# Deci-AI/super-gradients

Measured on NVIDIA H100. Metric: images/sec YOLO-NAS-S 640 bf16 train, higher is better.
Workload: dtype bf16

## Files before the change

### super_gradients_b200/csrc/conv_sm100.cu

```cuda
#include <cuda.h>

#include <cstdlib>
#include <cstring>

#include "common.cuh"
#include "conv_sm100.h"
#include "sm100_host.h"
#include "sm100_ptx.cuh"

namespace sm100 {

constexpr int BLOCK_M = 128;
constexpr int NUM_THREADS = 384;
constexpr int CONSUMER_THREADS = 256;
constexpr int MAX_STAGES = 8;

struct Params {
  int M;
  int N;
  int C;
  int KC;
  int n_tiles;
  int stages;
  int P, Q;
  int stride, pad;
  int b_cols_per_tap;
  int ntaps;
  signed char tap_dh[9], tap_dw[9], tap_b[9];
  int out_mode, o_mul, oh_add, ow_add, outH, outW;
  long long y_pitch;
  int y_off;
  bf16* y;
  const float* scale;
  const float* shift;
  const bf16* residual;
  double* stats;
  int stats_repl;
  int act;
};

__device__ __forceinline__ long long out_row(const Params& p, long long m) {
  if (p.out_mode == 0) return m;
  const int pq = p.P * p.Q;
  const int n = (int)(m / pq);
  const int rem = (int)(m - (long long)n * pq);
  const int j = rem / p.Q, i = rem - j * p.Q;
  return ((long long)n * p.outH + j * p.o_mul + p.oh_add) * p.outW + i * p.o_mul + p.ow_add;
}

__device__ __forceinline__ void consumer_sync() { asm volatile("bar.sync 1, %0;" ::"n"(CONSUMER_THREADS) : "memory"); }

constexpr uint32_t CTRL_BAR_BYTES = 16u * MAX_STAGES;

template <int BN>
__global__ void __launch_bounds__(NUM_THREADS, 1)
conv_wgmma_kernel(const __grid_constant__ CUtensorMap map_a, const __grid_constant__ CUtensorMap map_b, const Params p) {
  SGB_GRID_DEP_LAUNCH();
  extern __shared__ __align__(1024) unsigned char smem_raw[];
  const uint32_t smem_base = (smem_u32(smem_raw) + 1023u) & ~1023u;
  const uint32_t a_bytes = BLOCK_M * p.KC * 2, b_bytes = BN * p.KC * 2;
  const uint32_t stage_bytes = a_bytes + ((b_bytes + 1023u) & ~1023u);
  const uint32_t ctrl = smem_base + p.stages * stage_bytes;
  auto full_bar = [&](int s) { return ctrl + 8u * s; };
  auto empty_bar = [&](int s) { return ctrl + 8u * (MAX_STAGES + s); };
  float* s_part = reinterpret_cast<float*>(smem_raw + (ctrl + CTRL_BAR_BYTES - smem_u32(smem_raw)));
  float* s_stats = s_part + 8 * 2 * BN;

  const int warp = threadIdx.x >> 5, lane = threadIdx.x & 31;
  const int m_tiles = (p.M + BLOCK_M - 1) / BLOCK_M;
  const int total_tiles = m_tiles * p.n_tiles;
  const int chunks = (p.C + p.KC - 1) / p.KC;
  const int k_iters = p.ntaps * chunks;

  if (threadIdx.x == 0) {
    for (int s = 0; s < p.stages; ++s) {
      mbar_init(full_bar(s), 1);
      mbar_init(empty_bar(s), 8);
    }
    asm volatile("fence.mbarrier_init.release.cluster;" ::: "memory");
    asm volatile("fence.proxy.async.shared::cta;" ::: "memory");
  }
  if (p.stats)
    for (int i = threadIdx.x; i < 2 * p.N; i += NUM_THREADS) s_stats[i] = 0.f;
  __syncthreads();
  SGB_GRID_DEP_WAIT();

  if (warp == 0) {
    if (elect_one()) {
      int stg = 0;
      uint32_t par = 1;
      const int pq = p.P * p.Q;
// ... 75 lines not shown
        rrow[h] = p.residual ? p.residual + orow * p.y_pitch + p.y_off + n0 : nullptr;
      }
#pragma unroll
      for (int j = 0; j < BN / 8; ++j) {
        const int col = 8 * j + 2 * (lane & 3);
        const bool col_ok = col < ncols;
        float sum0 = 0.f, sum1 = 0.f, sq0 = 0.f, sq1 = 0.f;
#pragma unroll
        for (int h = 0; h < 2; ++h) {
          float v0 = acc[4 * j + 2 * h], v1 = acc[4 * j + 2 * h + 1];
          const bool ok = row_ok[h] && col_ok;
          if (p.scale && col_ok) {
            v0 *= p.scale[n0 + col];
            v1 *= p.scale[n0 + col + 1];
          }
          if (p.shift && col_ok) {
            v0 += p.shift[n0 + col];
            v1 += p.shift[n0 + col + 1];
          }
          if (rrow[h] && ok) {
            const uint32_t rr = *reinterpret_cast<const uint32_t*>(rrow[h] + col);
            v0 += __uint_as_float(rr << 16);
            v1 += __uint_as_float(rr & 0xffff0000u);
          }
          if (p.act != SGB_ACT_NONE) {
            v0 = apply_act(v0, p.act);
            v1 = apply_act(v1, p.act);
          }
          __nv_bfloat162 hh = __floats2bfloat162_rn(v0, v1);
          const uint32_t pk = *reinterpret_cast<uint32_t*>(&hh);
          if (ok) {
            *reinterpret_cast<uint32_t*>(yrow[h] + col) = pk;
            const float lo = __uint_as_float(pk << 16), hi = __uint_as_float(pk & 0xffff0000u);
            sum0 += lo;
            sum1 += hi;
            sq0 = fmaf(lo, lo, sq0);
            sq1 = fmaf(hi, hi, sq1);
          }
        }
        if (p.stats) {
#pragma unroll
          for (int o = 4; o < 32; o <<= 1) {
            sum0 += __shfl_xor_sync(0xffffffffu, sum0, o);
            sum1 += __shfl_xor_sync(0xffffffffu, sum1, o);
            sq0 += __shfl_xor_sync(0xffffffffu, sq0, o);
            sq1 += __shfl_xor_sync(0xffffffffu, sq1, o);
          }
          if (lane < 4) {
            float* part = s_part + (wg * 4 + wq) * 2 * BN;
            part[col] = sum0;
            part[col + 1] = sum1;
            part[BN + col] = sq0;
            part[BN + col + 1] = sq1;
          }
        }
      }
      if (p.stats) {
        consumer_sync();
        for (int i = threadIdx.x - 128; i < 2 * BN; i += CONSUMER_THREADS) {
          const int which = i / BN, c = i - which * BN;
          if (c < ncols) {
            float v = 0.f;
#pragma unroll
            for (int w = 0; w < 8; ++w) v += s_part[w * 2 * BN + i];
            s_stats[which * p.N + n0 + c] += v;
          }
        }
        consumer_sync();
      }
    }
  }
  __syncthreads();
  if (p.stats) {
    double* st = p.stats + (long long)(blockIdx.x & (p.stats_repl - 1)) * 2 * p.N;
    for (int i = threadIdx.x; i < 2 * p.N; i += NUM_THREADS) {
      const float v = s_stats[i];
      if (v != 0.f) atomicAdd(&st[i], (double)v);
    }
  }
}

struct WParams {
  int K, C;
  int R, S, stride, pad, P, Q;
  int npix;
  int CB;
  int n_ctiles, n_ktiles;
  int pix_per_cta;
  int stages;
  int cpad;
  float* dw;
};
constexpr int WPIX = 64;

template <int NB>
__global__ void __launch_bounds__(NUM_THREADS, 1)
wgrad_wgmma_kernel(const __grid_constant__ CUtensorMap map_dy, const __grid_constant__ CUtensorMap map_x, const WParams p) {
  SGB_GRID_DEP_LAUNCH();
  extern __shared__ __align__(1024) unsigned char smem_raw[];
  const uint32_t smem_base = (smem_u32(smem_raw) + 1023u) & ~1023u;
  const uint32_t a_bytes = 2 * WPIX * 128;
  const uint32_t b_box = WPIX * p.CB * 2;
  const int boxes = NB / p.CB;
  const uint32_t stage_bytes = a_bytes + (uint32_t)boxes * b_box;
  const uint32_t ctrl = smem_base + p.stages * stage_bytes;
  auto full_bar = [&](int s) { return ctrl + 8u * s; };
  auto empty_bar = [&](int s) { return ctrl + 8u * (MAX_STAGES + s); };

  const int warp = threadIdx.x >> 5, lane = threadIdx.x & 31;
  int w = blockIdx.x;
  const int ktile = w % p.n_ktiles; w /= p.n_ktiles;
  const int ctile = w % p.n_ctiles; w /= p.n_ctiles;
  const int tap = w % (p.R * p.S); w /= p.R * p.S;
  const int split = w;
  const int pix0 = split * p.pix_per_cta;
  const int pix1 = min(pix0 + p.pix_per_cta, p.npix);
  const int n_iters = (pix1 - pix0 + WPIX - 1) / WPIX;

  if (threadIdx.x == 0) {
    for (int s = 0; s < p.stages; ++s) {
      mbar_init(full_bar(s), 1);
      mbar_init(empty_bar(s), 8);
    }
    asm volatile("fence.mbarrier_init.release.cluster;" ::: "memory");
    asm volatile("fence.proxy.async.shared::cta;" ::: "memory");
  }
  __syncthreads();
  SGB_GRID_DEP_WAIT();

  if (n_iters > 0) {
    if (warp == 0) {
      if (elect_one()) {
        const int pq = p.P * p.Q;
        const int r = tap / p.S, s = tap - r * p.S;
        int stg = 0;
        uint32_t par = 1;
        for (int it = 0; it < n_iters; ++it) {
          mbar_wait(empty_bar(stg), par);
          const uint32_t sa = smem_base + stg * stage_bytes, sb = sa + a_bytes;
          mbar_expect_tx(full_bar(stg), a_bytes + (uint32_t)boxes * b_box);
          const int pix = pix0 + it * WPIX;
          tma_load_2d(sa, &map_dy, full_bar(stg), ktile * 128, pix);
          tma_load_2d(sa + WPIX * 128, &map_dy, full_bar(stg), ktile * 128 + 64, pix);
          const int n_img = pix / pq;
          const int rem = pix - n_img * pq;
          const int p0 = rem / p.Q, q0 = rem - p0 * p.Q;
          const int w0 = q0 * p.stride - p.pad, h0 = p0 * p.stride - p.pad;
          for (int bx = 0; bx < boxes; ++bx)
            tma_load_im2col_4d(sb + (uint32_t)bx * b_box, &map_x, full_bar(stg), ctile * NB + bx * p.CB, w0, h0, n_img, (uint16_t)s,
                               (uint16_t)r);
          if (++stg == p.stages) {
            stg = 0;
            par ^= 1;
          }
        }
      }
    } else if (warp >= 4) {
      const int wg = (warp >> 2) - 1, wq = warp & 3;
      const int b_row_bytes = p.CB * 2;
      float acc[NB / 2];
      int stg = 0, prev = -1;
      uint32_t par = 0;
      for (int it = 0; it < n_iters; ++it) {
        mbar_wait(full_bar(stg), par);
        const uint32_t sa = smem_base + stg * stage_bytes + (uint32_t)wg * (WPIX * 128), sb = smem_base + stg * stage_bytes + a_bytes;
        wgmma_fence();
#pragma unroll
        for (int j = 0; j < WPIX / 16; ++j) {
          const uint64_t da = smem_desc(sa + (uint32_t)j * 16u * 128u, 128, WPIX * 128, 8 * 128);
          const uint64_t db = smem_desc(sb + (uint32_t)j * 16u * (uint32_t)b_row_bytes, b_row_bytes, b_box, 8u * (uint32_t)b_row_bytes);
          mma_mn<NB>(acc, da, db, (it | j) != 0);
        }
        wgmma_commit();
        if (prev >= 0) {
          wgmma_wait<1>();
          __syncwarp();
          if (lane == 0) mbar_arrive(empty_bar(prev));
        }
        prev = stg;
        if (++stg == p.stages) {
          stg = 0;
          par ^= 1;
        }
      }
      wgmma_wait<0>();
      fence_regs(acc);
      const int row_len = p.R * p.S * p.cpad;
#pragma unroll
      for (int h = 0; h < 2; ++h) {
        const int ko = ktile * 128 + wg * 64 + wq * 16 + (lane >> 2) + 8 * h;
        if (ko < p.K) {
          float* drow = p.dw + (long long)ko * row_len + tap * p.cpad + ctile * NB + 2 * (lane & 3);
#pragma unroll
          for (int j = 0; j < NB / 8; ++j)
            asm volatile("red.global.add.v2.f32 [%0], {%1, %2};" ::"l"(drow + 8 * j), "f"(acc[4 * j + 2 * h]), "f"(acc[4 * j + 2 * h + 1])
                         : "memory");
        }
      }
    }
  }
}

EncodeTiledFn g_tiled = nullptr;
EncodeIm2colFn g_im2col = nullptr;
int g_num_sms = 0;
long long g_launches = 0;
long long launch_count() { return g_launches; }

int init_driver() {
  if (g_tiled && g_im2col) return SGB_OK;
  cudaDriverEntryPointQueryResult qres;
  void* fn = nullptr;
  if (cudaGetDriverEntryPoint("cuTensorMapEncodeTiled", &fn, cudaEnableDefault, &qres) != cudaSuccess || !fn) {
    sgb_set_error("cuTensorMapEncodeTiled entry point not found");
    return SGB_E_CUDA;
  }
  g_tiled = (EncodeTiledFn)fn;
  fn = nullptr;
  if (cudaGetDriverEntryPoint("cuTensorMapEncodeIm2col", &fn, cudaEnableDefault, &qres) != cudaSuccess || !fn) {
    sgb_set_error("cuTensorMapEncodeIm2col entry point not found");
    return SGB_E_CUDA;
  }
  g_im2col = (EncodeIm2colFn)fn;
  int dev = 0;
  cudaGetDevice(&dev);
  cudaDeviceGetAttribute(&g_num_sms, cudaDevAttrMultiProcessorCount, dev);
  return SGB_OK;
}

CUtensorMapSwizzle swizzle_for(int kc) {
  return kc == 64 ? CU_TENSOR_MAP_SWIZZLE_128B : (kc == 32 ? CU_TENSOR_MAP_SWIZZLE_64B : CU_TENSOR_MAP_SWIZZLE_32B);
}

bool enabled() {
  static int v = -1;
  if (v < 0) {
    const char* e = getenv("SGB_DISABLE_SM100");
    v = (e && e[0] == '1') ? 0 : 1;
  }
  return v == 1;
}

bool supported(const Problem& q) {
  if (!enabled()) return false;
  if (q.C % 16 != 0 || q.b_rows % 8 != 0) return false;
  if (!((q.R == 1 && q.S == 1) || (q.R == 3 && q.S == 3))) return false;
  if (q.stride != 1 && q.stride != 2) return false;
  if (q.a_pitch % 8 != 0 || q.y_pitch % 8 != 0 || q.y_off % 8 != 0) return false;
  if (((uintptr_t)q.a & 15) || ((uintptr_t)q.b & 15) || ((uintptr_t)q.y & 15)) return false;
  if ((long long)q.N * q.P * q.Q >= (1ll << 31)) return false;
  if (q.b_rows > 4096) return false;
  return true;
}

namespace {

template <class Fn>
struct Variant {
  int bn;
  Fn fn;
  int regs;
  bool ready;
};
typedef void (*ConvFn)(const CUtensorMap, const CUtensorMap, const Params);
typedef void (*WgradFn)(const CUtensorMap, const CUtensorMap, const WParams);
Variant<ConvFn> g_conv[] = {{16, conv_wgmma_kernel<16>, 0, false},   {32, conv_wgmma_kernel<32>, 0, false},
                            {48, conv_wgmma_kernel<48>, 0, false},   {64, conv_wgmma_kernel<64>, 0, false},
                            {96, conv_wgmma_kernel<96>, 0, false},   {128, conv_wgmma_kernel<128>, 0, false}};
Variant<WgradFn> g_wgrad[] = {{16, wgrad_wgmma_kernel<16>, 0, false}, {32, wgrad_wgmma_kernel<32>, 0, false},
                              {48, wgrad_wgmma_kernel<48>, 0, false}, {64, wgrad_wgmma_kernel<64>, 0, false},
                              {96, wgrad_wgmma_kernel<96>, 0, false}, {128, wgrad_wgmma_kernel<128>, 0, false}};

template <class Fn>
int prepare(Variant<Fn>& v, const char* what) {
  if (v.ready) return SGB_OK;
  if (int rc = sgb_cuda_check(cudaFuncSetAttribute(v.fn, cudaFuncAttributeMaxDynamicSharedMemorySize, 227 * 1024), what)) return rc;
  cudaFuncAttributes fa{};
  if (int rc = sgb_cuda_check(cudaFuncGetAttributes(&fa, v.fn), what)) return rc;
  v.regs = fa.numRegs;
  v.ready = true;
  return SGB_OK;
}

int pick_bn(int n) {
  for (int bn : {16, 32, 48, 64, 96, 128})
    if (n <= bn) return bn;
  int best = 128, best_waste = (n + 127) / 128 * 128 - n;
  for (int bn : {96, 64}) {
    const int waste = (n + bn - 1) / bn * bn - n;
    if (waste < best_waste) { best_waste = waste; best = bn; }
  }
  return best;
}

}

int launch(const Problem& q, cudaStream_t st) {
  if (int rc = init_driver()) return rc;
  Params p{};
  p.M = q.N * q.P * q.Q;
  p.N = q.b_rows;
  p.C = q.C;
  p.KC = q.C % 64 == 0 ? 64 : (q.C % 32 == 0 ? 32 : 16);
  if (p.KC < 64 && q.C > 32) p.KC = 64;
  const int bn = pick_bn(p.N);
  p.n_tiles = (p.N + bn - 1) / bn;
  p.P = q.P; p.Q = q.Q; p.stride = q.stride; p.pad = q.pad;
  if (q.ntaps > 0) {
    p.ntaps = q.ntaps;
    for (int t = 0; t < q.ntaps; ++t) { p.tap_dh[t] = (signed char)q.tap_dh[t]; p.tap_dw[t] = (signed char)q.tap_dw[t]; p.tap_b[t] = (signed char)q.tap_b[t]; }
  } else {
    p.ntaps = q.R * q.S;
    for (int t = 0; t < p.ntaps; ++t) {
      p.tap_dh[t] = (signed char)(t / q.S);
      p.tap_dw[t] = (signed char)(t % q.S);
      p.tap_b[t] = (signed char)(q.flip ? (p.ntaps - 1 - t) : t);
    }
  }
  if (p.ntaps > 9) return SGB_E_UNSUPPORTED;
  p.out_mode = q.out_mode; p.o_mul = q.o_mul; p.oh_add = q.oh_add; p.ow_add = q.ow_add; p.outH = q.outH; p.outW = q.outW;
  p.b_cols_per_tap = q.b_cols_per_tap;
  p.y = (bf16*)q.y; p.y_pitch = q.y_pitch; p.y_off = q.y_off;
  p.scale = q.scale; p.shift = q.shift; p.residual = (const bf16*)q.residual;
  p.stats = q.stats; p.stats_repl = q.stats_repl > 0 ? q.stats_repl : 1; p.act = q.act;
  Variant<ConvFn>* var = nullptr;
  for (auto& v : g_conv)
    if (v.bn == bn) var = &v;
  if (int rc = prepare(*var, "conv_wgmma_kernel")) return rc;
  const uint32_t a_bytes = BLOCK_M * p.KC * 2, b_bytes = ((uint32_t)(bn * p.KC * 2) + 1023u) & ~1023u;
  const uint32_t stage_bytes = a_bytes + b_bytes;
  const uint32_t ctrl_bytes = CTRL_BAR_BYTES + (p.stats ? (uint32_t)(8 * 2 * bn + 2 * p.N) * 4u : 0u);
  const int regs_alloc = ((var->regs + 7) / 8) * 8 * NUM_THREADS;
  int ctas_per_sm = 65536 / regs_alloc;
  if (ctas_per_sm > 2) ctas_per_sm = 2;
  if (ctas_per_sm < 1) ctas_per_sm = 1;
  int stages = 0;
  for (;; --ctas_per_sm) {
    const uint32_t budget = (ctas_per_sm == 1 ? 226u : 227u / ctas_per_sm - 1u) * 1024u;
    stages = budget > ctrl_bytes + 1024 ? (int)((budget - ctrl_bytes - 1024) / stage_bytes) : 0;
    if (stages > MAX_STAGES) stages = MAX_STAGES;
    if (stages >= 4 || ctas_per_sm == 1) break;
  }
  if (stages < 2) { sgb_set_error("conv_wgmma: tile does not fit shared memory"); return SGB_E_UNSUPPORTED; }
  p.stages = stages;
  const size_t smem = 1024 + (size_t)stages * stage_bytes + ctrl_bytes;

  alignas(64) CUtensorMap map_a, map_b;
  {
    cuuint64_t dims[4] = {(cuuint64_t)q.C, (cuuint64_t)q.W, (cuuint64_t)q.H, (cuuint64_t)q.N};
    cuuint64_t strides[3] = {(cuuint64_t)q.a_pitch * 2, (cuuint64_t)q.W * q.a_pitch * 2, (cuuint64_t)q.H * q.W * q.a_pitch * 2};
    int lower[2] = {-q.pad, -q.pad};
    int upper[2] = {q.pad - (q.S - 1), q.pad - (q.R - 1)};
    if (q.ntaps > 0) {
      lower[0] = lower[1] = 0;
      upper[0] = q.Q - q.W;
      upper[1] = q.P - q.H;
    }
    cuuint32_t estr[4] = {1, (cuuint32_t)q.stride, (cuuint32_t)q.stride, 1};
    CUresult r = g_im2col(&map_a, CU_TENSOR_MAP_DATA_TYPE_BFLOAT16, 4, const_cast<void*>(q.a), dims, strides, lower, upper,
                          (cuuint32_t)p.KC, (cuuint32_t)BLOCK_M, estr, CU_TENSOR_MAP_INTERLEAVE_NONE, swizzle_for(p.KC),
                          CU_TENSOR_MAP_L2_PROMOTION_L2_128B, CU_TENSOR_MAP_FLOAT_OOB_FILL_NONE);
    if (r != CUDA_SUCCESS) {
      sgb_set_error("cuTensorMapEncodeIm2col failed with %d (C=%d W=%d H=%d N=%d pitch=%d pad=%d upper=%d,%d stride=%d KC=%d)", (int)r,
                    q.C, q.W, q.H, q.N, q.a_pitch, q.pad, upper[0], upper[1], q.stride, p.KC);
      return SGB_E_CUDA;
    }
  }
  {
    cuuint64_t dims[2] = {(cuuint64_t)q.b_cols, (cuuint64_t)q.b_rows};
    cuuint64_t strides[1] = {(cuuint64_t)q.b_cols * 2};
    cuuint32_t box[2] = {(cuuint32_t)p.KC, (cuuint32_t)bn};
    cuuint32_t estr[2] = {1, 1};
    CUresult r = g_tiled(&map_b, CU_TENSOR_MAP_DATA_TYPE_BFLOAT16, 2, const_cast<void*>(q.b), dims, strides, box, estr,
                         CU_TENSOR_MAP_INTERLEAVE_NONE, swizzle_for(p.KC), CU_TENSOR_MAP_L2_PROMOTION_L2_128B,
                         CU_TENSOR_MAP_FLOAT_OOB_FILL_NONE);
    if (r != CUDA_SUCCESS) {
      sgb_set_error("cuTensorMapEncodeTiled(B) failed with %d (cols=%d rows=%d KC=%d BN=%d)", (int)r, q.b_cols, q.b_rows, p.KC, bn);
      return SGB_E_CUDA;
    }
  }
  const int m_tiles = (p.M + BLOCK_M - 1) / BLOCK_M;
  int grid = m_tiles * p.n_tiles;
  if (grid > g_num_sms * ctas_per_sm) grid = g_num_sms * ctas_per_sm;
  SGB_LAUNCH(var->fn, grid, NUM_THREADS, smem, st, map_a, map_b, p);
  ++g_launches;
  return sgb_cuda_check(cudaGetLastError(), "conv_wgmma_kernel");
}

bool wgrad_supported(const WgradProblem& q) {
  if (!enabled()) return false;
  if (q.C % 16 != 0 || q.K % 8 != 0) return false;
  if (!((q.R == 1 && q.S == 1) || (q.R == 3 && q.S == 3))) return false;
  if (q.pad != q.R / 2 || (q.stride != 1 && q.stride != 2)) return false;
  if (q.x_pitch % 8 != 0 || q.y_pitch % 8 != 0) return false;
  if (((uintptr_t)q.x & 15) || ((uintptr_t)q.dy & 15)) return false;
  if ((long long)q.N * q.P * q.Q >= (1ll << 31)) return false;
  return true;
}

int wgrad_launch(const WgradProblem& q, cudaStream_t st) {
  if (int rc = init_driver()) return rc;
  WParams p{};
  p.K = q.K; p.C = q.C; p.R = q.R; p.S = q.S; p.stride = q.stride; p.pad = q.pad; p.P = q.P; p.Q = q.Q;
  p.npix = q.N * q.P * q.Q;
  int nb = 16;
  for (int cand : {128, 96, 64, 48, 32})
    if (q.C % cand == 0) { nb = cand; break; }
  p.CB = nb % 64 == 0 ? 64 : (nb % 32 == 0 ? 32 : 16);
  p.n_ctiles = q.C / nb;
  p.n_ktiles = (q.K + 127) / 128;
  p.cpad = q.C;
  p.dw = q.dw;
  Variant<WgradFn>* var = nullptr;
  for (auto& v : g_wgrad)
    if (v.bn == nb) var = &v;
  if (int rc = prepare(*var, "wgrad_wgmma_kernel")) return rc;
  const uint32_t stage_bytes = 2 * WPIX * 128 + (uint32_t)(nb / p.CB) * WPIX * p.CB * 2;
  int stages = (int)((200 * 1024 - CTRL_BAR_BYTES - 1024) / stage_bytes);
  if (stages > MAX_STAGES) stages = MAX_STAGES;
  if (stages < 2) return SGB_E_UNSUPPORTED;
  p.stages = stages;
  const size_t smem = 1024 + (size_t)stages * stage_bytes + CTRL_BAR_BYTES;
  const int base_ctas = p.n_ktiles * p.n_ctiles * q.R * q.S;
  const int total_iters = (p.npix + WPIX - 1) / WPIX;
  int splits = (2 * g_num_sms + base_ctas - 1) / base_ctas;
  if (splits > total_iters / 8) splits = total_iters / 8;
  if (splits < 1) splits = 1;
  int iters_per = (total_iters + splits - 1) / splits;
  p.pix_per_cta = iters_per * WPIX;
  splits = (p.npix + p.pix_per_cta - 1) / p.pix_per_cta;

  alignas(64) CUtensorMap map_dy, map_x;
  {
    cuuint64_t dims[2] = {(cuuint64_t)q.K, (cuuint64_t)p.npix};
    cuuint64_t strides[1] = {(cuuint64_t)q.y_pitch * 2};
    cuuint32_t box[2] = {64, (cuuint32_t)WPIX};
    cuuint32_t estr[2] = {1, 1};
    CUresult r = g_tiled(&map_dy, CU_TENSOR_MAP_DATA_TYPE_BFLOAT16, 2, const_cast<void*>(q.dy), dims, strides, box, estr,
                         CU_TENSOR_MAP_INTERLEAVE_NONE, CU_TENSOR_MAP_SWIZZLE_128B, CU_TENSOR_MAP_L2_PROMOTION_L2_128B,
                         CU_TENSOR_MAP_FLOAT_OOB_FILL_NONE);
    if (r != CUDA_SUCCESS) { sgb_set_error("cuTensorMapEncodeTiled(dy) failed with %d", (int)r); return SGB_E_CUDA; }
  }
  {
    cuuint64_t dims[4] = {(cuuint64_t)q.C, (cuuint64_t)q.W, (cuuint64_t)q.H, (cuuint64_t)q.N};
    cuuint64_t strides[3] = {(cuuint64_t)q.x_pitch * 2, (cuuint64_t)q.W * q.x_pitch * 2, (cuuint64_t)q.H * q.W * q.x_pitch * 2};
    int lower[2] = {-q.pad, -q.pad};
    int upper[2] = {q.pad - (q.S - 1), q.pad - (q.R - 1)};
    cuuint32_t estr[4] = {1, (cuuint32_t)q.stride, (cuuint32_t)q.stride, 1};
    CUresult r = g_im2col(&map_x, CU_TENSOR_MAP_DATA_TYPE_BFLOAT16, 4, const_cast<void*>(q.x), dims, strides, lower, upper,
                          (cuuint32_t)p.CB, (cuuint32_t)WPIX, estr, CU_TENSOR_MAP_INTERLEAVE_NONE,
                          swizzle_for(p.CB), CU_TENSOR_MAP_L2_PROMOTION_L2_128B,
                          CU_TENSOR_MAP_FLOAT_OOB_FILL_NONE);
    if (r != CUDA_SUCCESS) { sgb_set_error("cuTensorMapEncodeIm2col(x, wgrad) failed with %d", (int)r); return SGB_E_CUDA; }
  }
  const int grid = base_ctas * splits;
  SGB_LAUNCH(var->fn, grid, NUM_THREADS, smem, st, map_dy, map_x, p);
  ++g_launches;
  return sgb_cuda_check(cudaGetLastError(), "wgrad_wgmma_kernel");
}

}
```

### super_gradients_b200/csrc/sm100_ptx.cuh

```cuda
#pragma once
#include <cuda.h>

#include "common.cuh"

namespace sm100 {

__device__ __forceinline__ void mbar_init(uint32_t bar, uint32_t count) {
  asm volatile("mbarrier.init.shared::cta.b64 [%0], %1;" ::"r"(bar), "r"(count));
}
__device__ __forceinline__ void mbar_expect_tx(uint32_t bar, uint32_t bytes) {
  asm volatile("mbarrier.arrive.expect_tx.shared::cta.b64 _, [%0], %1;" ::"r"(bar), "r"(bytes) : "memory");
}
__device__ __forceinline__ void mbar_arrive(uint32_t bar) {
  asm volatile("mbarrier.arrive.shared::cta.b64 _, [%0];" ::"r"(bar) : "memory");
}
__device__ __forceinline__ void mbar_wait(uint32_t bar, uint32_t parity) {
  asm volatile(
      "{\n"
      ".reg .pred p;\n"
      "WAIT_LOOP:\n"
      "mbarrier.try_wait.parity.shared::cta.b64 p, [%0], %1;\n"
      "@p bra DONE;\n"
      "bra WAIT_LOOP;\n"
      "DONE:\n"
      "}\n" ::"r"(bar),
      "r"(parity)
      : "memory");
}
__device__ __forceinline__ bool elect_one() {
  uint32_t pred;
  asm volatile(
      "{\n"
      ".reg .pred p;\n"
      "elect.sync _|p, 0xffffffff;\n"
      "selp.u32 %0, 1, 0, p;\n"
      "}\n"
      : "=r"(pred));
  return pred != 0;
}
__device__ __forceinline__ void tma_load_2d(uint32_t dst, const CUtensorMap* map, uint32_t bar, int c0, int c1) {
  asm volatile(
      "cp.async.bulk.tensor.2d.shared::cluster.global.mbarrier::complete_tx::bytes [%0], [%1, {%3, %4}], [%2];" ::"r"(dst),
      "l"(reinterpret_cast<uint64_t>(map)), "r"(bar), "r"(c0), "r"(c1)
      : "memory");
}
__device__ __forceinline__ void tma_load_im2col_4d(uint32_t dst, const CUtensorMap* map, uint32_t bar, int c, int w, int h,
                                                   int n, uint16_t off_w, uint16_t off_h) {
  asm volatile(
      "cp.async.bulk.tensor.4d.shared::cluster.global.im2col.mbarrier::complete_tx::bytes [%0], [%1, {%3, %4, %5, %6}], [%2], "
      "{%7, %8};" ::"r"(dst),
      "l"(reinterpret_cast<uint64_t>(map)), "r"(bar), "r"(c), "r"(w), "r"(h), "r"(n), "h"(off_w), "h"(off_h)
      : "memory");
}
__device__ __forceinline__ void wgmma_fence() { asm volatile("wgmma.fence.sync.aligned;" ::: "memory"); }
__device__ __forceinline__ void wgmma_commit() { asm volatile("wgmma.commit_group.sync.aligned;" ::: "memory"); }
template <int N>
__device__ __forceinline__ void wgmma_wait() {
  asm volatile("wgmma.wait_group.sync.aligned %0;" ::"n"(N) : "memory");
}
template <int R>
__device__ __forceinline__ void fence_regs(float (&d)[R]) {
#pragma unroll
  for (int i = 0; i < R; ++i) asm volatile("" : "+f"(d[i])::"memory");
}

template <int N>
__device__ __forceinline__ void mma_kk(float (&d)[N / 2], uint64_t da, uint64_t db, uint32_t accumulate);
template <int N>
__device__ __forceinline__ void mma_mn(float (&d)[N / 2], uint64_t da, uint64_t db, uint32_t accumulate);
template <>
__device__ __forceinline__ void mma_kk<16>(float (&d)[8], uint64_t da, uint64_t db, uint32_t accumulate) {
  asm volatile(
      "{\n.reg .pred p;\nsetp.ne.b32 p, %10, 0;\n"
      "wgmma.mma_async.sync.aligned.m64n16k16.f32.bf16.bf16 {%0,%1,%2,%3,%4,%5,%6,%7}, %8, %9, p, 1, 1, 0, 0;\n}\n"
      : "+f"(d[0]), "+f"(d[1]), "+f"(d[2]), "+f"(d[3]), "+f"(d[4]), "+f"(d[5]), "+f"(d[6]), "+f"(d[7])
      : "l"(da), "l"(db), "r"(accumulate));
}
template <>
__device__ __forceinline__ void mma_mn<16>(float (&d)[8], uint64_t da, uint64_t db, uint32_t accumulate) {
  asm volatile(
      "{\n.reg .pred p;\nsetp.ne.b32 p, %10, 0;\n"
      "wgmma.mma_async.sync.aligned.m64n16k16.f32.bf16.bf16 {%0,%1,%2,%3,%4,%5,%6,%7}, %8, %9, p, 1, 1, 1, 1;\n}\n"
      : "+f"(d[0]), "+f"(d[1]), "+f"(d[2]), "+f"(d[3]), "+f"(d[4]), "+f"(d[5]), "+f"(d[6]), "+f"(d[7])
      : "l"(da), "l"(db), "r"(accumulate));
}
template <>
__device__ __forceinline__ void mma_kk<32>(float (&d)[16], uint64_t da, uint64_t db, uint32_t accumulate) {
  asm volatile(
      "{\n.reg .pred p;\nsetp.ne.b32 p, %18, 0;\n"
      "wgmma.mma_async.sync.aligned.m64n32k16.f32.bf16.bf16 {%0,%1,%2,%3,%4,%5,%6,%7,%8,%9,%10,%11,%12,%13,%14,%15}, %16, %17, p, 1, 1, 0, 0;\n}\n"
      : "+f"(d[0]), "+f"(d[1]), "+f"(d[2]), "+f"(d[3]), "+f"(d[4]), "+f"(d[5]), "+f"(d[6]), "+f"(d[7]), "+f"(d[8]), "+f"(d[9]), "+f"(d[10]), "+f"(d[11]), "+f"(d[12]), "+f"(d[13]), "+f"(d[14]), "+f"(d[15])
      : "l"(da), "l"(db), "r"(accumulate));
}
template <>
__device__ __forceinline__ void mma_mn<32>(float (&d)[16], uint64_t da, uint64_t db, uint32_t accumulate) {
  asm volatile(
      "{\n.reg .pred p;\nsetp.ne.b32 p, %18, 0;\n"
      "wgmma.mma_async.sync.aligned.m64n32k16.f32.bf16.bf16 {%0,%1,%2,%3,%4,%5,%6,%7,%8,%9,%10,%11,%12,%13,%14,%15}, %16, %17, p, 1, 1, 1, 1;\n}\n"
      : "+f"(d[0]), "+f"(d[1]), "+f"(d[2]), "+f"(d[3]), "+f"(d[4]), "+f"(d[5]), "+f"(d[6]), "+f"(d[7]), "+f"(d[8]), "+f"(d[9]), "+f"(d[10]), "+f"(d[11]), "+f"(d[12]), "+f"(d[13]), "+f"(d[14]), "+f"(d[15])
      : "l"(da), "l"(db), "r"(accumulate));
}
template <>
__device__ __forceinline__ void mma_kk<48>(float (&d)[24], uint64_t da, uint64_t db, uint32_t accumulate) {
  asm volatile(
      "{\n.reg .pred p;\nsetp.ne.b32 p, %26, 0;\n"
      "wgmma.mma_async.sync.aligned.m64n48k16.f32.bf16.bf16 {%0,%1,%2,%3,%4,%5,%6,%7,%8,%9,%10,%11,%12,%13,%14,%15,%16,%17,%18,%19,%20,%21,%22,%23}, %24, %25, p, 1, 1, 0, 0;\n}\n"
      : "+f"(d[0]), "+f"(d[1]), "+f"(d[2]), "+f"(d[3]), "+f"(d[4]), "+f"(d[5]), "+f"(d[6]), "+f"(d[7]), "+f"(d[8]), "+f"(d[9]), "+f"(d[10]), "+f"(d[11]), "+f"(d[12]), "+f"(d[13]), "+f"(d[14]), "+f"(d[15]), "+f"(d[16]), "+f"(d[17]), "+f"(d[18]), "+f"(d[19]), "+f"(d[20]), "+f"(d[21]), "+f"(d[22]), "+f"(d[23])
      : "l"(da), "l"(db), "r"(accumulate));
}
template <>
__device__ __forceinline__ void mma_mn<48>(float (&d)[24], uint64_t da, uint64_t db, uint32_t accumulate) {
  asm volatile(
      "{\n.reg .pred p;\nsetp.ne.b32 p, %26, 0;\n"
      "wgmma.mma_async.sync.aligned.m64n48k16.f32.bf16.bf16 {%0,%1,%2,%3,%4,%5,%6,%7,%8,%9,%10,%11,%12,%13,%14,%15,%16,%17,%18,%19,%20,%21,%22,%23}, %24, %25, p, 1, 1, 1, 1;\n}\n"
      : "+f"(d[0]), "+f"(d[1]), "+f"(d[2]), "+f"(d[3]), "+f"(d[4]), "+f"(d[5]), "+f"(d[6]), "+f"(d[7]), "+f"(d[8]), "+f"(d[9]), "+f"(d[10]), "+f"(d[11]), "+f"(d[12]), "+f"(d[13]), "+f"(d[14]), "+f"(d[15]), "+f"(d[16]), "+f"(d[17]), "+f"(d[18]), "+f"(d[19]), "+f"(d[20]), "+f"(d[21]), "+f"(d[22]), "+f"(d[23])
      : "l"(da), "l"(db), "r"(accumulate));
}
template <>
__device__ __forceinline__ void mma_kk<64>(float (&d)[32], uint64_t da, uint64_t db, uint32_t accumulate) {
  asm volatile(
      "{\n.reg .pred p;\nsetp.ne.b32 p, %34, 0;\n"
      "wgmma.mma_async.sync.aligned.m64n64k16.f32.bf16.bf16 {%0,%1,%2,%3,%4,%5,%6,%7,%8,%9,%10,%11,%12,%13,%14,%15,%16,%17,%18,%19,%20,%21,%22,%23,%24,%25,%26,%27,%28,%29,%30,%31}, %32, %33, p, 1, 1, 0, 0;\n}\n"
      : "+f"(d[0]), "+f"(d[1]), "+f"(d[2]), "+f"(d[3]), "+f"(d[4]), "+f"(d[5]), "+f"(d[6]), "+f"(d[7]), "+f"(d[8]), "+f"(d[9]), "+f"(d[10]), "+f"(d[11]), "+f"(d[12]), "+f"(d[13]), "+f"(d[14]), "+f"(d[15]), "+f"(d[16]), "+f"(d[17]), "+f"(d[18]), "+f"(d[19]), "+f"(d[20]), "+f"(d[21]), "+f"(d[22]), "+f"(d[23]), "+f"(d[24]), "+f"(d[25]), "+f"(d[26]), "+f"(d[27]), "+f"(d[28]), "+f"(d[29]), "+f"(d[30]), "+f"(d[31])
      : "l"(da), "l"(db), "r"(accumulate));
}
template <>
__device__ __forceinline__ void mma_mn<64>(float (&d)[32], uint64_t da, uint64_t db, uint32_t accumulate) {
  asm volatile(
      "{\n.reg .pred p;\nsetp.ne.b32 p, %34, 0;\n"
      "wgmma.mma_async.sync.aligned.m64n64k16.f32.bf16.bf16 {%0,%1,%2,%3,%4,%5,%6,%7,%8,%9,%10,%11,%12,%13,%14,%15,%16,%17,%18,%19,%20,%21,%22,%23,%24,%25,%26,%27,%28,%29,%30,%31}, %32, %33, p, 1, 1, 1, 1;\n}\n"
      : "+f"(d[0]), "+f"(d[1]), "+f"(d[2]), "+f"(d[3]), "+f"(d[4]), "+f"(d[5]), "+f"(d[6]), "+f"(d[7]), "+f"(d[8]), "+f"(d[9]), "+f"(d[10]), "+f"(d[11]), "+f"(d[12]), "+f"(d[13]), "+f"(d[14]), "+f"(d[15]), "+f"(d[16]), "+f"(d[17]), "+f"(d[18]), "+f"(d[19]), "+f"(d[20]), "+f"(d[21]), "+f"(d[22]), "+f"(d[23]), "+f"(d[24]), "+f"(d[25]), "+f"(d[26]), "+f"(d[27]), "+f"(d[28]), "+f"(d[29]), "+f"(d[30]), "+f"(d[31])
      : "l"(da), "l"(db), "r"(accumulate));
}
template <>
__device__ __forceinline__ void mma_kk<96>(float (&d)[48], uint64_t da, uint64_t db, uint32_t accumulate) {
  asm volatile(
      "{\n.reg .pred p;\nsetp.ne.b32 p, %50, 0;\n"
      "wgmma.mma_async.sync.aligned.m64n96k16.f32.bf16.bf16 {%0,%1,%2,%3,%4,%5,%6,%7,%8,%9,%10,%11,%12,%13,%14,%15,%16,%17,%18,%19,%20,%21,%22,%23,%24,%25,%26,%27,%28,%29,%30,%31,%32,%33,%34,%35,%36,%37,%38,%39,%40,%41,%42,%43,%44,%45,%46,%47}, %48, %49, p, 1, 1, 0, 0;\n}\n"
      : "+f"(d[0]), "+f"(d[1]), "+f"(d[2]), "+f"(d[3]), "+f"(d[4]), "+f"(d[5]), "+f"(d[6]), "+f"(d[7]), "+f"(d[8]), "+f"(d[9]), "+f"(d[10]), "+f"(d[11]), "+f"(d[12]), "+f"(d[13]), "+f"(d[14]), "+f"(d[15]), "+f"(d[16]), "+f"(d[17]), "+f"(d[18]), "+f"(d[19]), "+f"(d[20]), "+f"(d[21]), "+f"(d[22]), "+f"(d[23]), "+f"(d[24]), "+f"(d[25]), "+f"(d[26]), "+f"(d[27]), "+f"(d[28]), "+f"(d[29]), "+f"(d[30]), "+f"(d[31]), "+f"(d[32]), "+f"(d[33]), "+f"(d[34]), "+f"(d[35]), "+f"(d[36]), "+f"(d[37]), "+f"(d[38]), "+f"(d[39]), "+f"(d[40]), "+f"(d[41]), "+f"(d[42]), "+f"(d[43]), "+f"(d[44]), "+f"(d[45]), "+f"(d[46]), "+f"(d[47])
      : "l"(da), "l"(db), "r"(accumulate));
}
// ... 41 lines not shown
```

Before: 749.4.

## Add planned wgrad kernel variants with multi-tap grouping and variable consumer warpgroups

Reworks the weight-gradient WGMMA kernel so one CTA can cover several 64-row K blocks and several filter taps per stage, with 1–3 consumer warpgroups and register rebalancing through setmaxnreg. A host-side planner uses a simple cost model to pick the variant, tap grouping, split count and stage count, favouring whole waves. The aim is to reuse the loaded dy tile across taps and K blocks, cut redundant TMA traffic and improve wave quantization for small-channel 3x3 layers. In exchange it adds many template instantiations and more planner complexity, and the cost model may choose poorly for some shapes.

Result: faster. 783.4 (median of 6 runs) (+4.5%).

```diff
diff --git a/super_gradients_b200/csrc/conv_sm100.cu b/super_gradients_b200/csrc/conv_sm100.cu
--- a/super_gradients_b200/csrc/conv_sm100.cu
+++ b/super_gradients_b200/csrc/conv_sm100.cu
@@ -7,6 +7,7 @@
 #include "conv_sm100.h"
 #include "sm100_host.h"
 #include "sm100_ptx.cuh"
+#include "wgrad_plan.h"
 
 namespace sm100 {
 
@@ -248,118 +249,154 @@
 
 struct WParams {
   int K, C;
-  int R, S, stride, pad, P, Q;
+  int S, stride, pad, P, Q;
   int npix;
   int CB;
-  int n_ctiles, n_ktiles;
-  int pix_per_cta;
+  int mblks, tg;
+  int n_mtiles, n_ctiles, n_groups, splits;
   int stages;
-  int cpad;
+  int row_len;
   float* dw;
 };
-constexpr int WPIX = 64;
-
-template <int NB>
-__global__ void __launch_bounds__(NUM_THREADS, 1)
+
+template <int NB, int UPW, int NC>
+__global__ void __launch_bounds__(128 * (NC + 1), 1)
 wgrad_wgmma_kernel(const __grid_constant__ CUtensorMap map_dy, const __grid_constant__ CUtensorMap map_x, const WParams p) {
   SGB_GRID_DEP_LAUNCH();
   extern __shared__ __align__(1024) unsigned char smem_raw[];
   const uint32_t smem_base = (smem_u32(smem_raw) + 1023u) & ~1023u;
-  const uint32_t a_bytes = 2 * WPIX * 128;
+  const uint32_t a_bytes = (uint32_t)p.mblks * (WPIX * 128);
   const uint32_t b_box = WPIX * p.CB * 2;
   const int boxes = NB / p.CB;
-  const uint32_t stage_bytes = a_bytes + (uint32_t)boxes * b_box;
+  const uint32_t tap_bytes = (uint32_t)boxes * b_box;
+  const uint32_t stage_bytes = a_bytes + (uint32_t)p.tg * tap_bytes;
   const uint32_t ctrl = smem_base + p.stages * stage_bytes;
   auto full_bar = [&](int s) { return ctrl + 8u * s; };
-  auto empty_bar = [&](int s) { return ctrl + 8u * (MAX_STAGES + s); };
+  auto empty_bar = [&](int s) { return ctrl + 8u * (WGRAD_MAX_STAGES + s); };
 
   const int warp = threadIdx.x >> 5, lane = threadIdx.x & 31;
   int w = blockIdx.x;
-  const int ktile = w % p.n_ktiles; w /= p.n_ktiles;
+  const int mtile = w % p.n_mtiles; w /= p.n_mtiles;
   const int ctile = w % p.n_ctiles; w /= p.n_ctiles;
-  const int tap = w % (p.R * p.S); w /= p.R * p.S;
+  const int group = w % p.n_groups; w /= p.n_groups;
   const int split = w;
-  const int pix0 = split * p.pix_per_cta;
-  const int pix1 = min(pix0 + p.pix_per_cta, p.npix);
-  const int n_iters = (pix1 - pix0 + WPIX - 1) / WPIX;
+  const long long ti = (p.npix + WPIX - 1) / WPIX;
+  const int it0 = (int)(ti * split / p.splits), it1 = (int)(ti * (split + 1) / p.splits);
+  const int n_iters = it1 - it0;
 
   if (threadIdx.x == 0) {
     for (int s = 0; s < p.stages; ++s) {
       mbar_init(full_bar(s), 1);
-      mbar_init(empty_bar(s), 8);
+      mbar_init(empty_bar(s), 4 * NC);
     }
     asm volatile("fence.mbarrier_init.release.cluster;" ::: "memory");
     asm volatile("fence.proxy.async.shared::cta;" ::: "memory");
   }
   __syncthreads();
   SGB_GRID_DEP_WAIT();
-
-  if (n_iters > 0) {
-    if (warp == 0) {
-      if (elect_one()) {
-        const int pq = p.P * p.Q;
-        const int r = tap / p.S, s = tap - r * p.S;
-        int stg = 0;
-        uint32_t par = 1;
-        for (int it = 0; it < n_iters; ++it) {
-          mbar_wait(empty_bar(stg), par);
-          const uint32_t sa = smem_base + stg * stage_bytes, sb = sa + a_bytes;
-          mbar_expect_tx(full_bar(stg), a_bytes + (uint32_t)boxes * b_box);
-          const int pix = pix0 + it * WPIX;
-          tma_load_2d(sa, &map_dy, full_bar(stg), ktile * 128, pix);
-          tma_load_2d(sa + WPIX * 128, &map_dy, full_bar(stg), ktile * 128 + 64, pix);
-          const int n_img = pix / pq;
-          const int rem = pix - n_img * pq;
-          const int p0 = rem / p.Q, q0 = rem - p0 * p.Q;
-          const int w0 = q0 * p.stride - p.pad, h0 = p0 * p.stride - p.pad;
+  if (n_iters <= 0) return;
+
+  if (warp < 4) {
+    if constexpr (NC == 3) setmaxnreg_dec<40>();
+    if (warp == 0 && elect_one()) {
+      int pix = it0 * WPIX;
+      int n_img = pix / (p.P * p.Q);
+      int p0 = (pix - n_img * p.P * p.Q) / p.Q;
+      int q0 = pix - (n_img * p.P + p0) * p.Q;
+      const int dp = WPIX / p.Q, dq = WPIX - dp * p.Q;
+      const int r_first = group * p.tg / p.S, s_first = group * p.tg - r_first * p.S;
+      int stg = 0;
+      uint32_t par = 1;
+      for (int it = it0; it < it1; ++it) {
+        mbar_wait(empty_bar(stg), par);
+        const uint32_t sa = smem_base + stg * stage_bytes, sb = sa + a_bytes;
+        mbar_expect_tx(full_bar(stg), stage_bytes);
+        for (int m = 0; m < p.mblks; ++m)
+          tma_load_2d(sa + (uint32_t)m * (WPIX * 128), &map_dy, full_bar(stg), (mtile * p.mblks + m) * 64, pix);
+        const int w0 = q0 * p.stride - p.pad, h0 = p0 * p.stride - p.pad;
+        int r = r_first, s = s_first;
+        for (int t = 0; t < p.tg; ++t) {
           for (int bx = 0; bx < boxes; ++bx)
-            tma_load_im2col_4d(sb + (uint32_t)bx * b_box, &map_x, full_bar(stg), ctile * NB + bx * p.CB, w0, h0, n_img, (uint16_t)s,
-                               (uint16_t)r);
-          if (++stg == p.stages) {
-            stg = 0;
-            par ^= 1;
-          }
-        }
-      }
-    } else if (warp >= 4) {
-      const int wg = (warp >> 2) - 1, wq = warp & 3;
-      const int b_row_bytes = p.CB * 2;
-      float acc[NB / 2];
-      int stg = 0, prev = -1;
-      uint32_t par = 0;
-      for (int it = 0; it < n_iters; ++it) {
-        mbar_wait(full_bar(stg), par);
-        const uint32_t sa = smem_base + stg * stage_bytes + (uint32_t)wg * (WPIX * 128), sb = smem_base + stg * stage_bytes + a_bytes;
-        wgmma_fence();
-#pragma unroll
-        for (int j = 0; j < WPIX / 16; ++j) {
-          const uint64_t da = smem_desc(sa + (uint32_t)j * 16u * 128u, 128, WPIX * 128, 8 * 128);
-          const uint64_t db = smem_desc(sb + (uint32_t)j * 16u * (uint32_t)b_row_bytes, b_row_bytes, b_box, 8u * (uint32_t)b_row_bytes);
-          mma_mn<NB>(acc, da, db, (it | j) != 0);
-        }
-        wgmma_commit();
-        if (prev >= 0) {
-          wgmma_wait<1>();
-          __syncwarp();
-          if (lane == 0) mbar_arrive(empty_bar(prev));
-        }
-        prev = stg;
+            tma_load_im2col_4d(sb + (uint32_t)t * tap_bytes + (uint32_t)bx * b_box, &map_x, full_bar(stg), ctile * NB + bx * p.CB, w0, h0,
+                               n_img, (uint16_t)s, (uint16_t)r);
+          if (++s == p.S) {
+            s = 0;
+            ++r;
+          }
+        }
+        pix += WPIX;
+        q0 += dq;
+        p0 += dp;
+        if (q0 >= p.Q) {
+          q0 -= p.Q;
+          ++p0;
+        }
+        while (p0 >= p.P) {
+          p0 -= p.P;
+          ++n_img;
+        }
         if (++stg == p.stages) {
           stg = 0;
           par ^= 1;
         }
       }
-      wgmma_wait<0>();
-      fence_regs(acc);
-      const int row_len = p.R * p.S * p.cpad;
+    }
+  } else {
+    if constexpr (NC == 3) setmaxnreg_inc<152>();
+    const int wg = (warp >> 2) - 1, wq = warp & 3;
+    const int b_row_bytes = p.CB * 2;
+    uint32_t a_off[UPW], b_off[UPW];
+#pragma unroll
+    for (int i = 0; i < UPW; ++i) {
+      const int u = wg + i * NC;
+      const int t = u / p.mblks, m = u - t * p.mblks;
+      a_off[i] = (uint32_t)m * (WPIX * 128);
+      b_off[i] = a_bytes + (uint32_t)t * tap_bytes;
+    }
+    float acc[UPW][NB / 2];
+    int stg = 0, prev = -1;
+    uint32_t par = 0;
+    for (int it = 0; it < n_iters; ++it) {
+      mbar_wait(full_bar(stg), par);
+      const uint32_t st0 = smem_base + stg * stage_bytes;
+      wgmma_fence();
+#pragma unroll
+      for (int i = 0; i < UPW; ++i) {
+#pragma unroll
+        for (int j = 0; j < WPIX / 16; ++j) {
+          const uint64_t da = smem_desc(st0 + a_off[i] + (uint32_t)j * 16u * 128u, 128, WPIX * 128, 8 * 128);
+          const uint64_t db = smem_desc(st0 + b_off[i] + (uint32_t)j * 16u * (uint32_t)b_row_bytes, b_row_bytes, b_box, 8u * (uint32_t)b_row_bytes);
+          mma_mn<NB>(acc[i], da, db, (it | j) != 0);
+        }
+      }
+      wgmma_commit();
+      if (prev >= 0) {
+        wgmma_wait<1>();
+        __syncwarp();
+        if (lane == 0) mbar_arrive(empty_bar(prev));
+      }
+      prev = stg;
+      if (++stg == p.stages) {
+        stg = 0;
+        par ^= 1;
+      }
+    }
+    wgmma_wait<0>();
+#pragma unroll
+    for (int i = 0; i < UPW; ++i) fence_regs(acc[i]);
+#pragma unroll
+    for (int i = 0; i < UPW; ++i) {
+      const int u = wg + i * NC;
+      const int t = u / p.mblks, m = u - t * p.mblks;
+      const int tap = group * p.tg + t;
 #pragma unroll
       for (int h = 0; h < 2; ++h) {
-        const int ko = ktile * 128 + wg * 64 + wq * 16 + (lane >> 2) + 8 * h;
+        const int ko = (mtile * p.mblks + m) * 64 + wq * 16 + (lane >> 2) + 8 * h;
         if (ko < p.K) {
-          float* drow = p.dw + (long long)ko * row_len + tap * p.cpad + ctile * NB + 2 * (lane & 3);
+          float* drow = p.dw + (long long)ko * p.row_len + tap * p.C + ctile * NB + 2 * (lane & 3);
 #pragma unroll
           for (int j = 0; j < NB / 8; ++j)
-            asm volatile("red.global.add.v2.f32 [%0], {%1, %2};" ::"l"(drow + 8 * j), "f"(acc[4 * j + 2 * h]), "f"(acc[4 * j + 2 * h + 1])
+            asm volatile("red.global.add.v2.f32 [%0], {%1, %2};" ::"l"(drow + 8 * j), "f"(acc[i][4 * j + 2 * h]), "f"(acc[i][4 * j + 2 * h + 1])
                          : "memory");
         }
       }
@@ -433,9 +470,12 @@
 Variant<ConvFn> g_conv[] = {{16, conv_wgmma_kernel<16>, 0, false},   {32, conv_wgmma_kernel<32>, 0, false},
                             {48, conv_wgmma_kernel<48>, 0, false},   {64, conv_wgmma_kernel<64>, 0, false},
                             {96, conv_wgmma_kernel<96>, 0, false},   {128, conv_wgmma_kernel<128>, 0, false}};
-Variant<WgradFn> g_wgrad[] = {{16, wgrad_wgmma_kernel<16>, 0, false}, {32, wgrad_wgmma_kernel<32>, 0, false},
-                              {48, wgrad_wgmma_kernel<48>, 0, false}, {64, wgrad_wgmma_kernel<64>, 0, false},
-                              {96, wgrad_wgmma_kernel<96>, 0, false}, {128, wgrad_wgmma_kernel<128>, 0, false}};
+Variant<WgradFn> g_wgrad[] = {
+#define SGB_WGRAD_VARIANT_ENTRY(nb, upw, nc) {nb, wgrad_wgmma_kernel<nb, upw, nc>, 0, false},
+    SGB_WGRAD_VARIANTS(SGB_WGRAD_VARIANT_ENTRY)
+#undef SGB_WGRAD_VARIANT_ENTRY
+};
+static_assert(sizeof(g_wgrad) / sizeof(g_wgrad[0]) == WGRAD_NUM_VARIANTS, "one kernel per planner variant");
 
 template <class Fn>
 int prepare(Variant<Fn>& v, const char* what) {
@@ -566,39 +606,27 @@
 
 int wgrad_launch(const WgradProblem& q, cudaStream_t st) {
   if (int rc = init_driver()) return rc;
+  const long long npix = (long long)q.N * q.P * q.Q;
+  WgradPlan plan;
+  if (!plan_wgrad(q.K, q.C, q.R, q.S, npix, g_num_sms, &plan)) {
+    sgb_set_error("wgrad_wgmma: no plan for C=%d K=%d", q.C, q.K);
+    return SGB_E_UNSUPPORTED;
+  }
+  Variant<WgradFn>& var = g_wgrad[plan.variant];
+  if (int rc = prepare(var, "wgrad_wgmma_kernel")) return rc;
   WParams p{};
-  p.K = q.K; p.C = q.C; p.R = q.R; p.S = q.S; p.stride = q.stride; p.pad = q.pad; p.P = q.P; p.Q = q.Q;
-  p.npix = q.N * q.P * q.Q;
-  int nb = 16;
-  for (int cand : {128, 96, 64, 48, 32})
-    if (q.C % cand == 0) { nb = cand; break; }
-  p.CB = nb % 64 == 0 ? 64 : (nb % 32 == 0 ? 32 : 16);
-  p.n_ctiles = q.C / nb;
-  p.n_ktiles = (q.K + 127) / 128;
-  p.cpad = q.C;
+  p.K = q.K; p.C = q.C; p.S = q.S; p.stride = q.stride; p.pad = q.pad; p.P = q.P; p.Q = q.Q;
+  p.npix = (int)npix;
+  p.CB = plan.cb;
+  p.mblks = plan.mb / 64; p.tg = plan.tg;
+  p.n_mtiles = plan.n_mtiles; p.n_ctiles = plan.n_ctiles; p.n_groups = plan.n_groups; p.splits = plan.splits;
+  p.stages = plan.stages;
+  p.row_len = q.R * q.S * q.C;
   p.dw = q.dw;
-  Variant<WgradFn>* var = nullptr;
-  for (auto& v : g_wgrad)
-    if (v.bn == nb) var = &v;
-  if (int rc = prepare(*var, "wgrad_wgmma_kernel")) return rc;
-  const uint32_t stage_bytes = 2 * WPIX * 128 + (uint32_t)(nb / p.CB) * WPIX * p.CB * 2;
-  int stages = (int)((200 * 1024 - CTRL_BAR_BYTES - 1024) / stage_bytes);
-  if (stages > MAX_STAGES) stages = MAX_STAGES;
-  if (stages < 2) return SGB_E_UNSUPPORTED;
-  p.stages = stages;
-  const size_t smem = 1024 + (size_t)stages * stage_bytes + CTRL_BAR_BYTES;
-  const int base_ctas = p.n_ktiles * p.n_ctiles * q.R * q.S;
-  const int total_iters = (p.npix + WPIX - 1) / WPIX;
-  int splits = (2 * g_num_sms + base_ctas - 1) / base_ctas;
-  if (splits > total_iters / 8) splits = total_iters / 8;
-  if (splits < 1) splits = 1;
-  int iters_per = (total_iters + splits - 1) / splits;
-  p.pix_per_cta = iters_per * WPIX;
-  splits = (p.npix + p.pix_per_cta - 1) / p.pix_per_cta;
 
   alignas(64) CUtensorMap map_dy, map_x;
   {
-    cuuint64_t dims[2] = {(cuuint64_t)q.K, (cuuint64_t)p.npix};
+    cuuint64_t dims[2] = {(cuuint64_t)q.K, (cuuint64_t)npix};
     cuuint64_t strides[1] = {(cuuint64_t)q.y_pitch * 2};
     cuuint32_t box[2] = {64, (cuuint32_t)WPIX};
     cuuint32_t estr[2] = {1, 1};
@@ -614,13 +642,12 @@
     int upper[2] = {q.pad - (q.S - 1), q.pad - (q.R - 1)};
     cuuint32_t estr[4] = {1, (cuuint32_t)q.stride, (cuuint32_t)q.stride, 1};
     CUresult r = g_im2col(&map_x, CU_TENSOR_MAP_DATA_TYPE_BFLOAT16, 4, const_cast<void*>(q.x), dims, strides, lower, upper,
-                          (cuuint32_t)p.CB, (cuuint32_t)WPIX, estr, CU_TENSOR_MAP_INTERLEAVE_NONE,
-                          swizzle_for(p.CB), CU_TENSOR_MAP_L2_PROMOTION_L2_128B,
+                          (cuuint32_t)plan.cb, (cuuint32_t)WPIX, estr, CU_TENSOR_MAP_INTERLEAVE_NONE,
+                          swizzle_for(plan.cb), CU_TENSOR_MAP_L2_PROMOTION_L2_128B,
                           CU_TENSOR_MAP_FLOAT_OOB_FILL_NONE);
     if (r != CUDA_SUCCESS) { sgb_set_error("cuTensorMapEncodeIm2col(x, wgrad) failed with %d", (int)r); return SGB_E_CUDA; }
   }
-  const int grid = base_ctas * splits;
-  SGB_LAUNCH(var->fn, grid, NUM_THREADS, smem, st, map_dy, map_x, p);
+  SGB_LAUNCH(var.fn, plan.grid, plan.threads, plan.smem, st, map_dy, map_x, p);
   ++g_launches;
   return sgb_cuda_check(cudaGetLastError(), "wgrad_wgmma_kernel");
 }
diff --git a/super_gradients_b200/csrc/sm100_ptx.cuh b/super_gradients_b200/csrc/sm100_ptx.cuh
--- a/super_gradients_b200/csrc/sm100_ptx.cuh
+++ b/super_gradients_b200/csrc/sm100_ptx.cuh
@@ -57,6 +57,14 @@
 template <int N>
 __device__ __forceinline__ void wgmma_wait() {
   asm volatile("wgmma.wait_group.sync.aligned %0;" ::"n"(N) : "memory");
+}
+template <int N>
+__device__ __forceinline__ void setmaxnreg_dec() {
+  asm volatile("setmaxnreg.dec.sync.aligned.u32 %0;" ::"n"(N));
+}
+template <int N>
+__device__ __forceinline__ void setmaxnreg_inc() {
+  asm volatile("setmaxnreg.inc.sync.aligned.u32 %0;" ::"n"(N));
 }
 template <int R>
 __device__ __forceinline__ void fence_regs(float (&d)[R]) {
diff --git a/super_gradients_b200/csrc/wgrad_plan.h b/super_gradients_b200/csrc/wgrad_plan.h
--- /dev/null
+++ b/super_gradients_b200/csrc/wgrad_plan.h
@@ -0,0 +1,128 @@
+#pragma once
+#include <cstdint>
+#include <initializer_list>
+
+namespace sm100 {
+
+constexpr int WPIX = 64;
+constexpr int WGRAD_MAX_STAGES = 8;
+constexpr int WGRAD_MAX_ACC = 96;
+constexpr uint32_t WGRAD_SMEM_BUDGET = 220u * 1024u;
+
+#define SGB_WGRAD_VARIANTS(X)                                                       \
+  X(16, 1, 1) X(32, 1, 1) X(48, 1, 1) X(64, 1, 1) X(96, 1, 1) X(128, 1, 1)      \
+  X(16, 1, 2) X(32, 1, 2) X(48, 1, 2) X(64, 1, 2) X(96, 1, 2) X(128, 1, 2)      \
+  X(16, 1, 3) X(32, 1, 3) X(48, 1, 3) X(64, 1, 3) X(96, 1, 3) X(128, 1, 3)      \
+  X(48, 2, 3) X(64, 2, 3) X(96, 2, 3)                                           \
+  X(32, 3, 3) X(48, 3, 3) X(64, 3, 3)
+
+struct WgradVariant {
+  int nb, upw, nc;
+};
+#define SGB_WGRAD_VARIANT_ROW(nb, upw, nc) {nb, upw, nc},
+constexpr WgradVariant WGRAD_VARIANTS[] = {SGB_WGRAD_VARIANTS(SGB_WGRAD_VARIANT_ROW)};
+#undef SGB_WGRAD_VARIANT_ROW
+constexpr int WGRAD_NUM_VARIANTS = sizeof(WGRAD_VARIANTS) / sizeof(WGRAD_VARIANTS[0]);
+
+struct WgradPlan {
+  int variant;
+  int nb, upw, nc;
+  int cb;
+  int mb, tg;
+  int n_mtiles, n_ctiles, n_groups;
+  int splits, grid, waves, stages, threads;
+  uint32_t stage_bytes, smem;
+  double staged_bytes;
+  double cost;
+};
+
+constexpr double WGRAD_L2_BPC = 32.0, WGRAD_SMEM_BPC = 128.0, WGRAD_MMA_FPC = 4096.0, WGRAD_CTA_FIXED = 3000.0;
+
+inline int wgrad_box_channels(int nb) { return nb % 64 == 0 ? 64 : (nb % 32 == 0 ? 32 : 16); }
+
+inline bool plan_wgrad(int K, int C, int R, int S, long long npix, int num_sms, WgradPlan* out) {
+  const int T = R * S;
+  const long long ti = (npix + WPIX - 1) / WPIX;
+  const long long max_splits = ti / 8 > 0 ? ti / 8 : 1;
+  const int kblocks = (K + 63) / 64;
+  bool found = false;
+  WgradPlan best{};
+  if (C % 16 != 0) return false;
+  if (!(R == 3 && C <= 96)) {
+    int nb = 16;
+    for (int cand : {128, 96, 64, 48, 32})
+      if (C % cand == 0) { nb = cand; break; }
+    const int mblks = kblocks % 2 == 0 ? 2 : (kblocks % 3 == 0 ? 3 : 1);
+    for (int v = 0; v < WGRAD_NUM_VARIANTS; ++v)
+      if (WGRAD_VARIANTS[v].nb == nb && WGRAD_VARIANTS[v].upw == 1 && WGRAD_VARIANTS[v].nc == mblks) best.variant = v;
+    best.nb = nb; best.upw = 1; best.nc = mblks; best.cb = wgrad_box_channels(nb);
+    best.mb = 64 * mblks; best.tg = 1;
+    best.n_mtiles = kblocks / mblks; best.n_ctiles = C / nb; best.n_groups = T;
+    const long long base = (long long)best.n_mtiles * best.n_ctiles * T;
+    long long splits = (2ll * num_sms + base - 1) / base;
+    if (splits > max_splits) splits = max_splits;
+    const long long iters = (ti + splits - 1) / splits;
+    splits = (ti + iters - 1) / iters;
+    best.splits = (int)splits; best.grid = (int)(base * splits); best.waves = (int)((base * splits + num_sms - 1) / num_sms);
+    best.stage_bytes = (uint32_t)(mblks * WPIX * 128 + WPIX * nb * 2);
+    best.stages = (int)((WGRAD_SMEM_BUDGET - 1024 - 16 * WGRAD_MAX_STAGES) / best.stage_bytes);
+    if (best.stages > WGRAD_MAX_STAGES) best.stages = WGRAD_MAX_STAGES;
+    best.threads = 128 * (mblks + 1);
+    best.smem = 1024u + (uint32_t)best.stages * best.stage_bytes + 16u * WGRAD_MAX_STAGES;
+    best.staged_bytes = (double)ti * WPIX * 2.0 * ((double)K * best.n_ctiles * T + (double)C * T * best.n_mtiles);
+    best.cost = 0;
+    *out = best;
+    return true;
+  }
+  for (int whole_waves = 1; whole_waves >= 0 && !found; --whole_waves)
+  for (int v = 0; v < WGRAD_NUM_VARIANTS; ++v) {
+    const WgradVariant& var = WGRAD_VARIANTS[v];
+    if (C % var.nb != 0 || var.upw * var.nb / 2 > WGRAD_MAX_ACC) continue;
+    const int units = var.upw * var.nc;
+    for (int tg : {1, S, T}) {
+      if (units % tg != 0) continue;
+      const int mblks = units / tg;
+      if (mblks > 3 || kblocks % mblks != 0) continue;
+      const int mb = 64 * mblks;
+      const int cb = wgrad_box_channels(var.nb);
+      const uint32_t stage_bytes = (uint32_t)(mblks * WPIX * 128 + tg * WPIX * var.nb * 2);
+      int stages = (int)((WGRAD_SMEM_BUDGET - 1024 - 16 * WGRAD_MAX_STAGES) / stage_bytes);
+      if (stages > WGRAD_MAX_STAGES) stages = WGRAD_MAX_STAGES;
+      if (stages < 3) continue;
+      const int n_mtiles = kblocks / mblks, n_ctiles = C / var.nb, n_groups = T / tg;
+      const long long base = (long long)n_mtiles * n_ctiles * n_groups;
+      const double staged = stage_bytes;
+      const double reads = (double)mblks * tg * (WPIX / 16) * (2048.0 + 32.0 * var.nb);
+      const double flops = (double)mblks * tg * 2.0 * 64 * var.nb * WPIX;
+      double it_cyc = staged / WGRAD_L2_BPC;
+      if ((staged + reads) / WGRAD_SMEM_BPC > it_cyc) it_cyc = (staged + reads) / WGRAD_SMEM_BPC;
+      if (flops / WGRAD_MMA_FPC > it_cyc) it_cyc = flops / WGRAD_MMA_FPC;
+      const double fixed = WGRAD_CTA_FIXED + (double)mb * tg * var.nb * 4 / WGRAD_L2_BPC;
+      for (long long splits = 1; splits <= max_splits; ++splits) {
+        const long long grid = base * splits;
+        if (grid > (1ll << 31) - 1) break;
+        const long long waves = (grid + num_sms - 1) / num_sms;
+        if (whole_waves && waves > 1 && 10 * (grid - (waves - 1) * num_sms) < 9ll * num_sms) continue;
+        const long long iters = (ti + splits - 1) / splits;
+        const double cost = (double)waves * (iters * it_cyc + fixed);
+        const double staged_total = (double)ti * WPIX * 2.0 * ((double)K * n_ctiles * n_groups + (double)C * T * n_mtiles);
+        if (found && !(cost < best.cost * 0.999 || (cost <= best.cost * 1.001 && staged_total < best.staged_bytes))) continue;
+        found = true;
+        best.variant = v;
+        best.nb = var.nb; best.upw = var.upw; best.nc = var.nc; best.cb = cb;
+        best.mb = mb; best.tg = tg;
+        best.n_mtiles = n_mtiles; best.n_ctiles = n_ctiles; best.n_groups = n_groups;
+        best.splits = (int)splits; best.grid = (int)grid; best.waves = (int)waves; best.stages = stages;
+        best.threads = 128 * (var.nc + 1);
+        best.stage_bytes = stage_bytes;
+        best.smem = 1024u + (uint32_t)stages * stage_bytes + 16u * WGRAD_MAX_STAGES;
+        best.staged_bytes = staged_total;
+        best.cost = cost;
+      }
+    }
+  }
+  if (found) *out = best;
+  return found;
+}
+
+}
```
